# SysCV/LiDAR_snow_sim

Measured on NVIDIA H100. Metric: augmented LiDAR points/sec, higher is better.
Workload: dtype f64

## Files before the change

### lidar_snow_sim_b200/csrc/beam.cuh

```cuda
#pragma once
#include "common.cuh"

struct __align__(16) SolveItem {
    unsigned long long key;
    int hit_off;
    int L;
    float th32;
    float px, py, pz;
};

struct DevArgs {
    const ParticleRec *rec;
    const ParticleTan *tan;
    const int64_t *plane_off;
    float zbase;
    const BroadEntry *entries;
    const int32_t *bucket_start;
    int n_buckets;
    int n_planes;
    double inv_w, w;
    const float *pts;
    const float *theta;
    const int64_t *cloud_off;
    const int32_t *order;
    const double *thresh;
    const SensorConst *sensor;
    const CameraConst *camera;
    const double *R;
    const double2 *wtab;
    double half_div;
    double div_rad;
    uint32_t flags;
    float *aug;
    float *keep_d;
    float *keep_i;
    uint8_t *keep_tag;
    uint8_t *code_keep;
    uint8_t *code_all;
    int32_t *nocc;
    unsigned *hist_keep;
    unsigned *hist_all;
    const int32_t *tile_base;
    double *stats;
    int *counters;
    unsigned *att_cnt;
    unsigned long long *att_sum;
    int *status;
    SolveItem *items;
    int *chunk_tab;
    int chunks_per_class;
    int *hdr;
    int *hit_idx;
    int hit_cap;
    const unsigned long long *sched;
    int n_wtiles;
};

namespace {

constexpr int SNOW_TPB = 128;
constexpr int SNOW_WARPS = SNOW_TPB / 32;
constexpr int TILE = 1024;
constexpr int NBINS = LSS_N_CHANNELS + 1;
constexpr int LIST_HDR_BYTES = 1024;
constexpr int LIST_CLASSES = 128;
constexpr int LIST_CHUNK = 1024;
constexpr int SCHED_PLANES = 64;
constexpr int SCHED_BINS = SCHED_PLANES + 1;

__device__ __forceinline__ void raise_status(int *status, int code) { atomicMax(status, code); }

__device__ __forceinline__ int channel_bin(float ch)
{
    int c = (int)ch;
    return (ch >= 0.0f && ch < 64.0f && (float)c == ch) ? c : LSS_N_CHANNELS;
}

__device__ __forceinline__ uint8_t keep_tag_of(int bin, float label)
{
    return (uint8_t)(bin + NBINS * (label == 2.0f ? 2 : (label == 1.0f ? 1 : 0)));
}

__device__ __forceinline__ int keep_tag_label(int tag) { return tag >= 2 * NBINS ? 2 : (tag >= NBINS ? 1 : 0); }

__device__ __forceinline__ bool within(double diff, double tol)
{
    return (fabs(diff) < tol) || (fabs(diff - LSS_TWO_PI) < tol) || (fabs(diff + LSS_TWO_PI) < tol);
}

__device__ __forceinline__ double xsi64(double r)
{
    if (r <= 0.9) return 0.0;
    if (r >= 1.0) return 1.0;
    const double m = (1 - 0) / (1.0 - 0.9);
    const double b = 0 - (m * 0.9);
    return __dadd_rn(__dmul_rn(m, r), b);
}

__device__ __forceinline__ double xsi32(float r)
{
    if (r <= 0.9f) return 0.0;
    if (r >= 1.0f) return 1.0;
    const double m = (1 - 0) / (1.0 - 0.9);
    const double b = 0 - (m * 0.9);
    return (double)__fadd_rn(__fmul_rn((float)m, r), (float)b);
}


__device__ __noinline__ float azimuth32_slow(float y, float x)
{
    return (float)atan2((double)y, (double)x);
}

__device__ const double ATAN_I32[33] = {
        0.0, 0.031239833430268277, 0.06241880999595735, 0.09347678115858947,
        0.12435499454676144, 0.15499674192394097, 0.18534794999569476, 0.21535769969773805,
        0.24497866312686414, 0.2741674511196588, 0.3028848683749714, 0.3310960767041321,
        0.35877067027057225, 0.38588266939807375, 0.4124104415973873, 0.43833655985795783,
        0.4636476090008061, 0.48833395105640554, 0.5123894603107377, 0.5358112379604637,
        0.5585993153435624, 0.5807563535676704, 0.6022873461349642, 0.6231993299340659,
        0.6435011087932844, 0.6632029927060933, 0.6823165548747481, 0.7008544078844502,
        0.7188299996216245, 0.7362574289814281, 0.7531512809621944, 0.7695264804056583,
        0.7853981633974483};

__device__ __forceinline__ float azimuth32(float yf, float xf)
{
    const float axf = fabsf(xf), ayf = fabsf(yf);
    const float mxf = fmaxf(axf, ayf), mnf = fminf(axf, ayf);
    if (!(mnf > 0.0f) || !(mxf < 3.0e38f) || !(mnf > mxf * 1e-30f) || xf != xf || yf != yf) return azimuth32_slow(yf, xf);
    const int i = (int)rintf(__fdividef(mnf, mxf) * 32.0f);
    const double c = (double)i * (1.0 / 32.0), mx = (double)mxf, mn = (double)mnf;
    const double t = fma(-c, mx, mn) / fma(c, mn, mx);
    const double t2 = t * t;
    double p = fma(t2, 1.0 / 9.0, -1.0 / 7.0);
    p = fma(t2, p, 1.0 / 5.0);
// ... 17 lines not shown
```

### lidar_snow_sim_b200/csrc/snowfall.cu

```cuda
#include "beam.cuh"

namespace {

constexpr int SCHED_KEY_TPB = 128;

__global__ void __launch_bounds__(SCHED_KEY_TPB) k_sched_key(const float *__restrict__ pts, const int64_t *__restrict__ cloud_off,
                                                            const int32_t *__restrict__ order, const int32_t *__restrict__ wtile_base,
                                                            unsigned long long *ent, int *hist)
{
    const int b = blockIdx.y, t = blockIdx.x * SCHED_KEY_TPB + threadIdx.x;
    const int64_t beg = cloud_off[b];
    const int n = (int)(cloud_off[b + 1] - beg);
    if (blockIdx.x * SCHED_KEY_TPB * 32 >= n) return;
    const int w0 = 32 * t;
    const bool on = w0 < n;
    int bin = -1;
    if (on) {
        const int ch = channel_bin(pts[(beg + w0) * 5 + 4]);
        bin = ch < LSS_N_CHANNELS ? order[b * LSS_N_CHANNELS + ch] % SCHED_PLANES : SCHED_PLANES;
        ent[wtile_base[b] + t] = ((unsigned long long)bin << 48) | ((unsigned long long)b << 32) | (unsigned)w0;
    }
    const unsigned m = __match_any_sync(0xffffffffu, bin);
    if (on && (threadIdx.x & 31) == __ffs(m) - 1) atomicAdd(&hist[bin], __popc(m));
}

constexpr int HIT_POS_PER_BEAM = 6;
constexpr int SCHED_PER_THREAD = 2;
__global__ void __launch_bounds__(256) k_sched_sort(const unsigned long long *__restrict__ in, unsigned long long *out,
                                                    int *hist, int n)
{
    __shared__ int base[SCHED_BINS], cnt[SCHED_BINS], blk[SCHED_BINS];
    const int first = blockIdx.x * (256 * SCHED_PER_THREAD);
    for (int c = threadIdx.x; c < SCHED_BINS; c += 256) cnt[c] = 0;
    if (threadIdx.x < 32) {
        int run = 0;
        for (int c0 = 0; c0 < SCHED_BINS; c0 += 32) {
            const int c = c0 + (int)threadIdx.x;
            const int v = c < SCHED_BINS ? hist[c] : 0;
            int incl = v;
#pragma unroll
            for (int s = 1; s < 32; s <<= 1) {
                const int t = __shfl_up_sync(0xffffffffu, incl, s);
                if ((int)threadIdx.x >= s) incl += t;
            }
            if (c < SCHED_BINS) base[c] = run + incl - v;
            run += __shfl_sync(0xffffffffu, incl, 31);
        }
    }
    __syncthreads();
    const int lane = threadIdx.x & 31;
    int bin_of[SCHED_PER_THREAD], rank[SCHED_PER_THREAD];
    unsigned long long e[SCHED_PER_THREAD];
#pragma unroll
    for (int k = 0; k < SCHED_PER_THREAD; k++) {
        const int s = first + k * 256 + threadIdx.x;
        const bool on = s < n;
        e[k] = on ? in[s] : 0ull;
        const int bin = on ? (int)(e[k] >> 48) : -1;
        bin_of[k] = bin;
        const unsigned m = __match_any_sync(0xffffffffu, bin);
        const int leader = __ffs(m) - 1;
        int r = 0;
        if (on && lane == leader) r = atomicAdd(&cnt[bin], __popc(m));
        r = __shfl_sync(0xffffffffu, r, leader);
        rank[k] = r + __popc(m & ((1u << lane) - 1u));
    }
    __syncthreads();
    for (int c = threadIdx.x; c < SCHED_BINS; c += 256)
        blk[c] = cnt[c] ? atomicAdd(&hist[SCHED_BINS + c], cnt[c]) : 0;
    __syncthreads();
#pragma unroll
    for (int k = 0; k < SCHED_PER_THREAD; k++)
        if (bin_of[k] >= 0) out[base[bin_of[k]] + blk[bin_of[k]] + rank[k]] = e[k];
}

constexpr int KEEP_TPB = 256;
constexpr int KEEP_ROWS = TILE / KEEP_TPB;

__global__ void __launch_bounds__(KEEP_TPB) k_keep(DevArgs a)
{
    __shared__ unsigned h_keep[NBINS], h_all[NBINS];
    __shared__ int s_cnt[2];
    const int b = blockIdx.y, tile = blockIdx.x;
    const int64_t beg = a.cloud_off[b];
    const int n = (int)(a.cloud_off[b + 1] - beg);
    if (tile * TILE >= n) return;
    if (threadIdx.x < NBINS) { h_keep[threadIdx.x] = 0; h_all[threadIdx.x] = 0; }
    if (threadIdx.x < 2) s_cnt[threadIdx.x] = 0;
    const bool thr_on = a.flags & LSS_FLAG_THRESHOLD_FILTER;
    int tags[KEEP_ROWS];
    float d32s[KEEP_ROWS], out_is[KEEP_ROWS];
#pragma unroll
    for (int k = 0; k < KEEP_ROWS; k++) {
        const int i = tile * TILE + k * KEEP_TPB + threadIdx.x;
        tags[k] = 0; d32s[k] = 0.0f; out_is[k] = 0.0f;
        if (i < n) {
            tags[k] = __ldcs(a.keep_tag + beg + i);
            if (thr_on) { d32s[k] = __ldcs(a.keep_d + beg + i); out_is[k] = __ldcs(a.keep_i + beg + i); }
        }
    }
    double p0 = 0.0, p1 = 0.0, p2 = 0.0;
    if (thr_on) { p0 = a.thresh[3 * b]; p1 = a.thresh[3 * b + 1]; p2 = a.thresh[3 * b + 2]; }
    __syncthreads();
    const int lane = threadIdx.x & 31;
#pragma unroll
    for (int k = 0; k < KEEP_ROWS; k++) {
        const int i = tile * TILE + k * KEEP_TPB + threadIdx.x;
        const bool active = i < n;
        bool keep = false, att = false;
// ... 78 lines not shown
            run += __shfl_sync(0xffffffffu, incl, 31);
        }
        if (lane == 0) bin_total[c] = run;
    }
    __syncthreads();
    if (threadIdx.x == 0) {
        unsigned run = 0;
        for (int c = 0; c < NBINS; c++) { const unsigned t = bin_total[c]; bin_total[c] = run; run += t; }
        if (counts) counts[b] = (int32_t)run;
        if (stats) {
            const int n_att = counters[2 * b], n_rem = counters[2 * b + 1];
            double sum = 0.0;
            for (int c = 0; c < LSS_N_CHANNELS; c++) sum += att_term[c];
            sum -= (double)att_sum[b];
            stats[4 * b + 3] = sum;
            stats[4 * b + 0] = (double)n_att;
            stats[4 * b + 1] = (double)n_rem;
            stats[4 * b + 2] = n_att > 0 ? (double)(long long)(sum / (double)n_att) : 0.0;
        }
    }
    __syncthreads();
    const int total = n_tiles * NBINS;
    for (int k0 = threadIdx.x; k0 < total; k0 += TSCAN_ADD * blockDim.x) {
        unsigned v[TSCAN_ADD];
#pragma unroll
        for (int q = 0; q < TSCAN_ADD; q++) {
            const int k = k0 + q * blockDim.x;
            v[q] = k < total ? h[k] : 0u;
        }
#pragma unroll
        for (int q = 0; q < TSCAN_ADD; q++) {
            const int k = k0 + q * blockDim.x;
            if (k < total) h[k] = v[q] + bin_total[k % NBINS];
        }
    }
}

__global__ void __launch_bounds__(TILE) k_scatter(const float *__restrict__ aug, const uint8_t *__restrict__ code,
                                                   const unsigned *__restrict__ tile_off,
                                                   const int64_t *__restrict__ cloud_off,
                                                   const int32_t *__restrict__ tile_base,
                                                   float *__restrict__ out, const int32_t *__restrict__ nocc_in,
                                                   int32_t *__restrict__ nocc_out, int32_t *__restrict__ perm_out)
{
    __shared__ unsigned warp_cnt[TILE / 32][NBINS];
    const int b = blockIdx.y, tile = blockIdx.x;
    const int64_t beg = cloud_off[b];
    const int n = (int)(cloud_off[b + 1] - beg);
    const int i = tile * TILE + threadIdx.x;
    if (tile * TILE >= n) return;
    const int lane = threadIdx.x & 31, warp = threadIdx.x >> 5;
    for (int k = threadIdx.x; k < (TILE / 32) * NBINS; k += TILE) (&warp_cnt[0][0])[k] = 0;
    __syncthreads();
    int c = -1;
    if (i < n) {
        const int cc = code[beg + i];
        c = cc < NBINS ? cc : -1;
    }
    const unsigned m = __match_any_sync(0xffffffffu, c);
    const int rank = __popc(m & ((1u << lane) - 1u));
    if (c >= 0 && rank == 0) warp_cnt[warp][c] = __popc(m);
    __syncthreads();
    if (threadIdx.x < NBINS) {
        unsigned run = tile_off[((size_t)tile_base[b] + tile) * NBINS + threadIdx.x];
        for (int wv = 0; wv < TILE / 32; wv++) { const unsigned t = warp_cnt[wv][threadIdx.x]; warp_cnt[wv][threadIdx.x] = run; run += t; }
    }
    __syncthreads();
    if (c >= 0) {
        const int64_t dst = beg + warp_cnt[warp][c] + rank;
        const float *s = aug + (beg + i) * 5;
        float *o = out + dst * 5;
#pragma unroll
        for (int q = 0; q < 5; q++) o[q] = s[q];
        if (nocc_out) nocc_out[dst] = nocc_in[beg + i];
        if (perm_out) perm_out[dst] = i;
    }
}

struct WsLayout {
    int64_t aug, keep_d, keep_i, keep_tag, code_keep, code_all, nocc, hist_keep, hist_all, hist_rows, cloud_off, tile_base,
        order, thresh, counters, counters_bytes, list, chunks_per_class, chunk_tab, sched, sched_tiles, prepass, prepass_bytes, total;
};

WsLayout ws_layout(int64_t n_total, int n_clouds)
{
    WsLayout w;
    w.hist_rows = n_total / TILE + (int64_t)n_clouds + 1;
    w.sched_tiles = n_total / 32 + (int64_t)n_clouds + 1;
    int64_t o = 0;
    w.aug = o;        o = align_up(o + n_total * 5 * 4, 256);
    w.keep_d = o;     o = align_up(o + n_total * 4, 256);
    w.keep_i = o;     o = align_up(o + n_total * 4, 256);
    w.keep_tag = o;   o = align_up(o + n_total, 256);
    w.code_keep = o;  o = align_up(o + n_total, 256);
    w.code_all = o;   o = align_up(o + n_total, 256);
    w.nocc = o;       o = align_up(o + n_total * 4, 256);
    w.hist_keep = o;  o = align_up(o + w.hist_rows * NBINS * 4, 256);
    w.hist_all = o;   o = align_up(o + w.hist_rows * NBINS * 4, 256);
    w.cloud_off = o;  o = align_up(o + (int64_t)(n_clouds + 1) * 8, 256);
    w.tile_base = o;  o = align_up(o + (int64_t)(n_clouds + 1) * 2 * 4, 256);
    w.order = o;      o = align_up(o + (int64_t)n_clouds * LSS_N_CHANNELS * 4, 256);
    w.thresh = o;     o = align_up(o + (int64_t)n_clouds * 3 * 8, 256);
    w.counters_bytes = align_up((int64_t)n_clouds * 2 * 4, 8) + (int64_t)n_clouds * LSS_N_CHANNELS * 4 + (int64_t)n_clouds * 8;
    w.counters = o;   o = align_up(o + w.counters_bytes, 256);
    w.chunks_per_class = (n_total + LIST_CHUNK - 1) / LIST_CHUNK;
    w.list = o;       o = align_up(o + LIST_HDR_BYTES +
                                   (w.chunks_per_class + LIST_CLASSES) * LIST_CHUNK * (int64_t)sizeof(SolveItem) +
                                   (n_total * HIT_POS_PER_BEAM + 4096) * 4, 256);
    w.chunk_tab = o;  o = align_up(o + (int64_t)LIST_CLASSES * w.chunks_per_class * 4, 256);
    w.sched = o;      o = align_up(o + (int64_t)SCHED_BINS * 2 * 4 + 2 * w.sched_tiles * 8, 256);
    w.prepass_bytes = lss_prepass_ws_bytes(n_total, n_clouds);
    w.prepass = o;    o = align_up(o + w.prepass_bytes, 256);
    w.total = o;
    return w;
}

}

int64_t lss_snowfall_ws_bytes(int64_t n_total, int n_clouds)
{
    if (n_total < 0 || n_clouds < 0) return -1;
    return ws_layout(n_total, n_clouds).total;
}

int64_t lss_snowfall_ws_cloud_off(int64_t n_total, int n_clouds) { return ws_layout(n_total, n_clouds).cloud_off; }

lss_status lss_snowfall_run(lss_engine *e, const SnowfallArgs &s, cudaStream_t stream)
{
    const int B = s.n_clouds;
    BatchGeometry g, wg;
    if (lss_status rc = lss_batch_geometry(e, s.h_cloud_offsets, B, TILE, g)) return rc;
    if (lss_status rc = lss_batch_geometry(e, s.h_cloud_offsets, B, 32, wg)) return rc;
    const int64_t N = g.n, max_n = g.max_n;
    for (int k = 0; k < B * LSS_N_CHANNELS; k++)
        if (s.h_order[k] < 0 || s.h_order[k] >= s.ts->n_planes)
            return lss_fail(e, LSS_ERR_NO_TABLE, "order[] names a plane that is not in the table set");
    const WsLayout w = ws_layout(N, B);
    if (s.workspace_bytes < w.total || !s.d_workspace) return lss_fail(e, LSS_ERR_WORKSPACE, "workspace too small");
    if ((s.flags & LSS_FLAG_THRESHOLD_FILTER) && !s.h_thresh_poly && !(s.flags & LSS_FLAG_DEVICE_PREPASS))
        return lss_fail(e, LSS_ERR_INVALID_ARG, "threshold filter needs h_thresh_poly or LSS_FLAG_DEVICE_PREPASS");
    if ((s.flags & LSS_FLAG_CAMERA_FOV) && !e->has_camera)
        return lss_fail(e, LSS_ERR_NO_SENSOR, "camera calibration not set");
    const double div_rad = s.beam_divergence_deg * (LSS_PI / 180.0);
    if (!(div_rad > 0) || div_rad > s.ts->max_div_rad * (1 + 1e-12))
        return lss_fail(e, LSS_ERR_INVALID_ARG, "beam_divergence exceeds the value the table set was built for");
    const int max_tiles = (int)((max_n + TILE - 1) / TILE);
    const int n_wtiles = wg.tile_base[B];
    if ((s.d_out_perm || s.d_out_nocc) && !s.d_out_full)
        return lss_fail(e, LSS_ERR_INVALID_ARG, "d_out_perm / d_out_nocc need d_out_full");

    char *ws = (char *)s.d_workspace;
    float *d_aug = (float *)(ws + w.aug);
    uint8_t *d_code_keep = (uint8_t *)(ws + w.code_keep);
    const bool want_all = s.d_out_full != nullptr;
    uint8_t *d_code_all = want_all ? (uint8_t *)(ws + w.code_all) : nullptr;
    int32_t *d_nocc_tmp = s.d_out_nocc ? (int32_t *)(ws + w.nocc) : nullptr;
    unsigned *d_hist_keep = (unsigned *)(ws + w.hist_keep);
    unsigned *d_hist_all = want_all ? (unsigned *)(ws + w.hist_all) : nullptr;
    int64_t *d_off = (int64_t *)(ws + w.cloud_off);
    int32_t *d_tile_base = (int32_t *)(ws + w.tile_base);
    int32_t *d_order = (int32_t *)(ws + w.order);
    double *d_thresh = (double *)(ws + w.thresh);
    int *d_counters = (int *)(ws + w.counters);
    unsigned *d_att_cnt = (unsigned *)(ws + w.counters + align_up((int64_t)B * 2 * 4, 8));
    unsigned long long *d_att_sum = (unsigned long long *)((char *)d_att_cnt + (int64_t)B * LSS_N_CHANNELS * 4);

    g.tile_base.insert(g.tile_base.end(), wg.tile_base.begin(), wg.tile_base.end());
    LSS_CUDA_CHECK(e, lss_stage_geometry(e, s.h_cloud_offsets, B, g.tile_base, d_off, d_tile_base, stream));
    LSS_CUDA_CHECK(e, lss_stage_upload(e, d_order, s.h_order, sizeof(int32_t) * B * LSS_N_CHANNELS, stream));
    if (s.h_thresh_poly)
        LSS_CUDA_CHECK(e, lss_stage_upload(e, d_thresh, s.h_thresh_poly, sizeof(double) * 3 * B, stream));
    int *d_list_hdr = (int *)(ws + w.list);
    {
        ZeroRegions z;
        z.add(d_counters, w.counters_bytes);
        z.add(s.d_out_stats, sizeof(double) * 4 * B);
        if (N == 0 || B == 0) {
            z.add(s.d_out_counts, sizeof(int32_t) * B);
            LSS_CUDA_CHECK(e, lss_zero_async(e, z, stream));
            return LSS_OK;
        }
        z.add(d_list_hdr, LIST_HDR_BYTES);
        z.add(ws + w.chunk_tab, (size_t)LIST_CLASSES * w.chunks_per_class * 4);
        z.add(ws + w.sched, (size_t)SCHED_BINS * 2 * 4);
        LSS_CUDA_CHECK(e, lss_zero_async(e, z, stream));
    }

    DevArgs a;
    a.rec = s.ts->d_rec;
    a.tan = s.ts->d_tan;
    a.plane_off = s.ts->d_plane_off;
    a.zbase = s.ts->zbase;
    a.entries = s.ts->d_entries;
    a.bucket_start = s.ts->d_bucket_start;
    a.n_buckets = s.ts->n_buckets;
    a.n_planes = s.ts->n_planes;
    a.w = LSS_TWO_PI / s.ts->n_buckets;
    a.inv_w = s.ts->n_buckets / LSS_TWO_PI;
    a.pts = s.d_points;
    a.theta = s.d_theta;
    a.cloud_off = d_off;
    a.order = d_order;
    a.thresh = d_thresh;
    a.sensor = e->d_sensor;
    a.camera = e->d_camera;
    a.R = e->d_R;
    a.wtab = e->d_wtab;
    a.half_div = (s.beam_divergence_deg / 2) * (LSS_PI / 180.0);
    a.div_rad = div_rad;
    a.flags = s.flags;
    a.aug = d_aug;
    a.keep_d = (float *)(ws + w.keep_d);
    a.keep_i = (float *)(ws + w.keep_i);
    a.keep_tag = (uint8_t *)(ws + w.keep_tag);
    a.code_keep = d_code_keep;
    a.code_all = d_code_all;
    a.nocc = d_nocc_tmp;
    a.hist_keep = d_hist_keep;
    a.hist_all = d_hist_all;
    a.tile_base = d_tile_base;
    a.stats = s.d_out_stats;
    a.counters = d_counters;
    a.att_cnt = d_att_cnt;
    a.att_sum = d_att_sum;
    a.status = e->d_status;
    SolveItem *d_solve_list = (SolveItem *)(ws + w.list + LIST_HDR_BYTES);
    a.hit_idx = (int *)(d_solve_list + (w.chunks_per_class + LIST_CLASSES) * LIST_CHUNK);
    const bool device_prepass = (s.flags & LSS_FLAG_THRESHOLD_FILTER) && (s.flags & LSS_FLAG_DEVICE_PREPASS) &&
                                !s.h_thresh_poly;
    cudaEvent_t ev_join = nullptr;
    if (device_prepass) {
        cudaStream_t side = nullptr;
        cudaEvent_t ev_fork = nullptr;
        LSS_CUDA_CHECK(e, lss_side_stream(e, &side, &ev_fork, &ev_join));
        LSS_CUDA_CHECK(e, cudaEventRecord(ev_fork, stream));
        LSS_CUDA_CHECK(e, cudaStreamWaitEvent(side, ev_fork, 0));
        PrepassIO io;
        io.h_plane_in = s.h_plane_in;
        io.h_ymins_in = s.h_ymins_in;
        io.d_poly_out = d_thresh;
        lss_status ps = lss_prepass_run(e, s.d_points, d_off, nullptr, s.h_cloud_offsets, B, 0.5, s.noise_floor, 0, 0, 1,
                                io, ws + w.prepass, w.prepass_bytes, nullptr, side);
        const cudaError_t je = cudaEventRecord(ev_join, side);
        if (ps != LSS_OK || je != cudaSuccess) {
            cudaStreamWaitEvent(stream, ev_join, 0);
            return ps != LSS_OK ? ps : lss_fail(e, LSS_ERR_CUDA, "event record failed");
        }
    }
    a.hit_cap = (int)std::min<int64_t>(N * HIT_POS_PER_BEAM + 4096, 0x7fffffff);
    cudaError_t ce;
    {
        KernelTimer kt(e, LSS_K_SNOWFALL, stream);
        a.hdr = d_list_hdr;
        a.items = d_solve_list;
        a.chunk_tab = (int *)(ws + w.chunk_tab);
        a.chunks_per_class = (int)w.chunks_per_class;
        {
            int *d_sched_hist = (int *)(ws + w.sched);
            unsigned long long *d_ent = (unsigned long long *)(d_sched_hist + 2 * SCHED_BINS);
            unsigned long long *d_sched = d_ent + w.sched_tiles;
            const int max_wtiles = (int)((max_n + 31) / 32);
            ce = lss_launch(e, k_sched_key, dim3((unsigned)((max_wtiles + SCHED_KEY_TPB - 1) / SCHED_KEY_TPB), (unsigned)B),
                            SCHED_KEY_TPB, 0, stream, s.d_points, d_off, d_order, d_tile_base + B + 1, d_ent, d_sched_hist);
            if (ce == cudaSuccess)
                ce = lss_launch(e, k_sched_sort, (unsigned)((n_wtiles + 256 * SCHED_PER_THREAD - 1) / (256 * SCHED_PER_THREAD)),
                                256, 0, stream, d_ent, d_sched, d_sched_hist, n_wtiles);
            a.sched = d_sched;
            a.n_wtiles = n_wtiles;
        }
        if (ce == cudaSuccess) {
            KernelTimer ks(e, LSS_K_SCAN, stream);
            ce = lss_launch_scan(e, a, stream);
        }
        if (ce == cudaSuccess) {
            KernelTimer ks(e, LSS_K_SOLVE, stream);
            ce = lss_launch_solve(e, a, d_list_hdr + 1, stream);
        }
    }
    if (ev_join) LSS_CUDA_CHECK(e, cudaStreamWaitEvent(stream, ev_join, 0));
    LSS_CUDA_CHECK(e, ce);
    {
        KernelTimer kt(e, LSS_K_FINALIZE, stream);
        LSS_CUDA_CHECK(e, lss_launch(e, k_keep, dim3(max_tiles, B), KEEP_TPB, 0, stream, a));
    }
    {
        KernelTimer kt(e, LSS_K_SORT, stream);
        LSS_CUDA_CHECK(e, lss_launch(e, k_tile_scan, B, 1024, 0, stream, d_hist_keep, d_tile_base, s.d_out_counts,
                                     s.d_out_stats, d_counters, d_att_cnt, d_att_sum, e->d_sensor));
    }
    {
        KernelTimer kt(e, LSS_K_COMPACT, stream);
        LSS_CUDA_CHECK(e, lss_launch(e, k_scatter, dim3(max_tiles, B), TILE, 0, stream, d_aug, d_code_keep, d_hist_keep, d_off,
                                     d_tile_base, s.d_out_points, nullptr, nullptr, nullptr));
    }
    if (want_all) {
        KernelTimer kt(e, LSS_K_COMPACT, stream);
        LSS_CUDA_CHECK(e, lss_launch(e, k_tile_scan, B, 1024, 0, stream, d_hist_all, d_tile_base, nullptr, nullptr, nullptr,
                                     nullptr, nullptr, nullptr));
        LSS_CUDA_CHECK(e, lss_launch(e, k_scatter, dim3(max_tiles, B), TILE, 0, stream, d_aug, d_code_all, d_hist_all, d_off,
                                     d_tile_base, s.d_out_full, d_nocc_tmp, s.d_out_nocc, s.d_out_perm));
    }
    return LSS_OK;
}
```

### lidar_snow_sim_b200/csrc/solve.cu

```cuda
#include "beam.cuh"

namespace {

constexpr int SOLVE_TPB = 128;
constexpr int SOLVE_WARPS = SOLVE_TPB / 32;
#ifndef LSS_SOLVE_CTAS
#define LSS_SOLVE_CTAS 5
#endif
#ifndef LSS_SOLVE_ARENA
#define LSS_SOLVE_ARENA 160
#endif
constexpr int SOLVE_CTAS_PER_SM = LSS_SOLVE_CTAS;
constexpr int ARENA = LSS_SOLVE_ARENA;
constexpr int SOLVE_LCAP = 128;
static_assert(SOLVE_LCAP + 1 <= ARENA, "a beam with SOLVE_LCAP occluders must fit a round of the arena on its own");
constexpr unsigned FULL = 0xffffffffu;

struct Beam {
    double d, right, left;
    bool straddle;
};

__device__ __forceinline__ void beam_limits(float th32, double half_div, Beam &bm)
{
    const double thd = (double)th32;
    double right = thd - half_div, left = thd + half_div;
    if (right < 0) right += LSS_TWO_PI;
    if (left < 0) left += LSS_TWO_PI;
    if (right > LSS_TWO_PI) right -= LSS_TWO_PI;
    if (left > LSS_TWO_PI) left -= LSS_TWO_PI;
    bm.right = right; bm.left = left; bm.straddle = right > left;
}

__device__ __forceinline__ bool exact_hit(const ParticleRec *rp, const Beam &bm, double &rho, bool &right_hit, bool &left_hit)
{
    rho = rp->rho;
    if (!(rho < bm.d)) return false;
    const double phi = rp->phi, alpha = rp->alpha;
    bool inside = (bm.right <= phi) && (phi <= bm.left);
    if (bm.straddle) inside = inside || ((bm.right - LSS_TWO_PI <= phi) && (phi <= bm.left)) ||
                              ((bm.right <= phi) && (phi <= bm.left + LSS_TWO_PI));
    right_hit = within(bm.right - phi, alpha);
    left_hit = within(bm.left - phi, alpha);
    return inside || right_hit || left_hit;
}

struct Bucket {
    int e0, e1;
    float th_rel;
    long long pbase;
};

__device__ __forceinline__ Bucket beam_bucket(const DevArgs &a, int plane, float th32)
{
    const double thd = (double)th32;
    const double thm = thd >= LSS_TWO_PI ? thd - LSS_TWO_PI : thd;
    int bk = (int)(thm * a.inv_w);
    bk = bk < 0 ? 0 : (bk >= a.n_buckets ? a.n_buckets - 1 : bk);
    const int32_t *bs = a.bucket_start + (int64_t)plane * (a.n_buckets + 1) + bk;
    Bucket k;
    k.e0 = bs[0];
    k.e1 = bs[1];
    k.th_rel = (float)(thm - (bk + 0.5) * a.w);
    k.pbase = a.plane_off[plane];
    return k;
}

template <class F>
__device__ __forceinline__ int for_each_hit(const DevArgs &a, const Bucket &k, const Beam &bm, float d32, F &&f)
{
    int n = 0;
#pragma unroll 1
    for (int e = k.e0; e < k.e1; e++) {
        const EntryView en = lss_decode(__ldg(&a.entries[e]), a.zbase);
        if (!(en.x < d32)) break;
        if (!(fabsf(en.y - k.th_rel) <= en.z)) continue;
        const long long pi = k.pbase + en.idx;
        double rho;
        bool rh, lh;
        if (exact_hit(a.rec + pi, bm, rho, rh, lh)) { f((int)pi, rho, rh, lh); n++; }
    }
    return n;
}

constexpr int SURV_CAP = 20;

__device__ __forceinline__ double shfl_f64(double v, int src)
{
    const long long b = __double_as_longlong(v);
    const int lo = __shfl_sync(FULL, (int)(unsigned)b, src), hi = __shfl_sync(FULL, (int)(b >> 32), src);
    return __longlong_as_double(((long long)hi << 32) | (unsigned)lo);
}

#ifndef LSS_SCAN_CTAS
#define LSS_SCAN_CTAS 10
#endif
__global__ void __launch_bounds__(SNOW_TPB, LSS_SCAN_CTAS) k_scan(DevArgs a)
{
    __shared__ float s_rows[SNOW_WARPS][32 * 5];
    __shared__ int s_idx[SNOW_WARPS][32][SURV_CAP];
    __shared__ unsigned s_hit[SNOW_WARPS][32];
    const int lane = threadIdx.x & 31, wid = threadIdx.x >> 5;
    const int st = blockIdx.x * SNOW_WARPS + wid;
    if (st >= a.n_wtiles) return;
    const unsigned long long se = a.sched[st];
    const int b = (int)((se >> 32) & 0xffffu), w0 = (int)(unsigned)se;
    const int64_t beg = a.cloud_off[b];
    const int n = (int)(a.cloud_off[b + 1] - beg);
    const int i = w0 + lane;
    const bool active = i < n;
    const int nf_w = min(32, n - w0) * 5;
    float px = 0, py = 0, pz = 0, pint = 0, pch = 0;
    {
        const float *src = a.pts + (beg + w0) * 5;
#pragma unroll
        for (int q = 0; q < 5; q++) {
            const int f = q * 32 + lane;
            if (f < nf_w) s_rows[wid][f] = __ldcs(src + f);
        }
        __syncwarp();
        if (active) {
            const float *row = &s_rows[wid][5 * lane];
            px = row[0]; py = row[1]; pz = row[2]; pint = row[3]; pch = row[4];
        }
    }
    const float d32 = __fsqrt_rn(__fadd_rn(__fadd_rn(__fmul_rn(px, px), __fmul_rn(py, py)), __fmul_rn(pz, pz)));
    const int ch = channel_bin(pch);
    float out_l = pch;
    int ns = 0;
    Bucket bkt;
    bkt.e0 = bkt.e1 = 0; bkt.th_rel = 0.0f; bkt.pbase = 0;
    bool slow = false;
    float th32 = 0.0f;
    Beam bm;
    bm.d = (double)d32; bm.right = bm.left = 0.0; bm.straddle = false;
    if (active && ch < LSS_N_CHANNELS) {
        out_l = 0.0f;
        th32 = a.theta ? a.theta[beg + i] : azimuth32(py, px);
        if (th32 < 0.0f) th32 = __fadd_rn(th32, 6.2831855f);
        beam_limits(th32, a.half_div, bm);
        const int plane = a.order[b * LSS_N_CHANNELS + ch];
        if (plane >= 0 && plane < a.n_planes && th32 == th32) {
            bkt = beam_bucket(a, plane, th32);
            const int e1 = bkt.e1;
            int *pos = s_idx[wid][lane];
            bool stop = false;
#pragma unroll 1
            for (int e = bkt.e0; e < e1 && !stop; e += 4) {
                BroadEntry raw[4];
#pragma unroll
                for (int q = 0; q < 4; q++) raw[q] = __ldg(&a.entries[min(e + q, e1 - 1)]);
#pragma unroll
                for (int q = 0; q < 4; q++) {
                    if (stop || e + q >= e1) continue;
                    const EntryView en = lss_decode(raw[q], a.zbase);
                    if (!(en.x < d32)) { stop = true; continue; }
                    if (!(fabsf(en.y - bkt.th_rel) <= en.z)) continue;
                    if (ns < SURV_CAP) pos[ns] = en.idx;
                    else slow = true;
                    ns++;
                }
            }
        }
    }
    s_hit[wid][lane] = 0u;
    const int mine = slow ? 0 : ns;
    int incl = mine;
#pragma unroll
    for (int sft = 1; sft < 32; sft <<= 1) {
        const int t = __shfl_up_sync(FULL, incl, sft);
        if (lane >= sft) incl += t;
    }
    const int off = incl - mine;
    const int total = __shfl_sync(FULL, incl, 31);
    __syncwarp();
#pragma unroll 1
    for (int s0 = 0; s0 < total; s0 += 32) {
        const int s = s0 + lane;
        int j = 0;
#pragma unroll
        for (int step = 16; step; step >>= 1) {
            const int c = j + step;
            const int oc = __shfl_sync(FULL, off, c & 31);
            if (c < 32 && oc <= s) j = c;
        }
        const int r = s - __shfl_sync(FULL, off, j);
        const long long pbj = __shfl_sync(FULL, bkt.pbase, j);
        Beam bj;
        bj.d = shfl_f64(bm.d, j);
        bj.right = shfl_f64(bm.right, j);
        bj.left = shfl_f64(bm.left, j);
        bj.straddle = bj.right > bj.left;
        if (s < total) {
            double rho;
            bool rh, lh;
            if (exact_hit(a.rec + pbj + s_idx[wid][j][r], bj, rho, rh, lh)) atomicOr(&s_hit[wid][j], 1u << r);
        }
    }
    __syncwarp();
    unsigned hits = s_hit[wid][lane];
    int L = __popc(hits);
    if (slow) L = for_each_hit(a, bkt, bm, d32, [](int, double, bool, bool) {});
    {
        const bool push = L > 0;
        const unsigned pm = __ballot_sync(FULL, push);
        int lincl = push ? L : 0;
#pragma unroll
        for (int sft = 1; sft < 32; sft <<= 1) {
            const int t = __shfl_up_sync(FULL, lincl, sft);
            if (lane >= sft) lincl += t;
        }
        const int ltotal = __shfl_sync(FULL, lincl, 31);
        if (pm) {
            int hbase = 0;
            const int leader = __ffs(pm) - 1;
            if (lane == leader) hbase = atomicAdd(a.hdr + 2, ltotal);
            hbase = __shfl_sync(FULL, hbase, leader);
            if (push) {
                const int cls = LIST_CLASSES - 1 - min(LIST_CLASSES - 1, 2 * min(L, 63) + (d32 > 40.0f ? 1 : 0));
                const unsigned cm = __match_any_sync(pm, cls);
                const int cl = __ffs(cm) - 1;
                int j = 0;
                if (lane == cl) j = atomicAdd(a.hdr + LIST_CLASSES + cls, __popc(cm));
                j = __shfl_sync(cm, j, cl) + __popc(cm & ((1u << lane) - 1u));
                int *ct = a.chunk_tab + (int64_t)cls * a.chunks_per_class + j / LIST_CHUNK;
                if (j % LIST_CHUNK == 0) atomicExch(ct, atomicAdd(a.hdr, 1) + 1);
                __syncwarp(pm);
                int chunk;
                while ((chunk = *(volatile int *)ct) == 0) {}
                const int hoff = hbase + lincl - L;
                const bool fits = hoff + L <= a.hit_cap;
                {
                    SolveItem it;
                    it.key = ((unsigned long long)ch << 56) | ((unsigned long long)cls << 48) |
                             ((unsigned long long)b << 32) | (unsigned)i;
                    it.hit_off = fits ? hoff : -1;
                    it.L = L;
                    it.th32 = th32;
                    it.px = px;
                    it.py = py;
                    it.pz = pz;
                    a.items[(int64_t)(chunk - 1) * LIST_CHUNK + j % LIST_CHUNK] = it;
                }
                if (fits) {
                    int *hp = a.hit_idx + hoff;
                    if (!slow) {
                        const int *pos = s_idx[wid][lane];
#pragma unroll 1
                        for (int k = 0; hits; hits &= hits - 1) hp[k++] = (int)bkt.pbase + pos[__ffs(hits) - 1];
                    } else {
                        for_each_hit(a, bkt, bm, d32, [&](int pi, double, bool, bool) { *hp++ = pi; });
                    }
                }
            }
        }
    }
    __syncwarp();
    if (active) {
        float *row = &s_rows[wid][5 * lane];
        const float out_i = rintf(pint);
        row[3] = out_i;
        row[4] = out_l;
        if (a.nocc) a.nocc[beg + i] = 0;
        a.keep_d[beg + i] = d32;
        a.keep_i[beg + i] = out_i;
        a.keep_tag[beg + i] = (uint8_t)ch;
    }
    __syncwarp();
    {
        float *dst = a.aug + (beg + w0) * 5;
#pragma unroll
        for (int q = 0; q < 5; q++) {
            const int f = q * 32 + lane;
            if (f < nf_w) dst[f] = s_rows[wid][f];
        }
    }
}

__device__ __forceinline__ unsigned long long pack_win(int ks, int ke, int k0)
{
    return (unsigned long long)(unsigned)ks | ((unsigned long long)(unsigned)ke << 11) | ((unsigned long long)(unsigned)k0 << 22);
}

__device__ __forceinline__ void pulse_phase(double r, double &sb, double &cb)
{
    const double ctau = 299792458.0 * 1e-8, inv_ctau = 1.0 / (299792458.0 * 1e-8);
    const double bh = r * inv_ctau;
    const double bl = fma(-bh, ctau, r) * inv_ctau;
    double s, c;
    sincospi(bh, &s, &c);
    const double corr = LSS_PI * bl;
    sb = fma(corr, c, s);
    cb = fma(-corr, s, c);
}

__device__ __forceinline__ void cp_async4(void *dst, const void *src)
{
    asm volatile("cp.async.ca.shared.global [%0], [%1], 4;\n" ::"r"((unsigned)__cvta_generic_to_shared(dst)), "l"(src) : "memory");
}
__device__ __forceinline__ void cp_async8(void *dst, const void *src)
{
    asm volatile("cp.async.ca.shared.global [%0], [%1], 8;\n" ::"r"((unsigned)__cvta_generic_to_shared(dst)), "l"(src) : "memory");
}
__device__ __forceinline__ void cp_async_wait_all() { asm volatile("cp.async.wait_all;\n" ::: "memory"); }

#ifdef LSS_SOLVE_PHASE_CLOCKS
enum { PH_FETCH, PH_FILL, PH_CLAIM, PH_PULSES, PH_SWEEP, PH_EVAL, PH_STORE, PH_N };
static_assert(PH_N + 2 + LIST_CLASSES == LSS_DEBUG_SOLVE_PHASE_WORDS, "layout of lss_debug_solve_phases");
__device__ unsigned long long g_solve_phase[LSS_DEBUG_SOLVE_PHASE_WORDS];
#define PHASE_INIT()                                                                                                  \
    __shared__ unsigned long long s_ph[SOLVE_WARPS][PH_N + 1];                                                        \
    if (lane <= PH_N) s_ph[wid][lane] = 0ull;                                                                         \
    unsigned ph_t = (unsigned)clock64();                         \
    unsigned ph_split = 0u
#define PHASE(k)                                                                                                      \
    do {                                                                                                              \
        const unsigned ph_n = (unsigned)clock64();                                                                    \
        if (lane == 0) s_ph[wid][k] += ph_n - ph_t;                                                                   \
        ph_t = ph_n;                                                                                                  \
    } while (0)
#define PHASE_MARK() (ph_split = (unsigned)clock64() - ph_t)
#define PHASE_SPLIT(k0, k1)                                                                                           \
    do {                                                                                                              \
        const unsigned ph_n = (unsigned)clock64();                                                                    \
        const unsigned sp = __reduce_max_sync(FULL, ph_split);                                                        \
        if (lane == 0) { s_ph[wid][k0] += sp; s_ph[wid][k1] += ph_n - ph_t - sp; }                                   \
        ph_t = ph_n;                                                                                                  \
        ph_split = 0u;                                                                                                \
    } while (0)
#define PHASE_TILE(cls, active)                                                                                       \
    do {                                                                                                              \
        const unsigned nb = __popc(__ballot_sync(FULL, active));                                                      \
        if (lane == 0) { s_ph[wid][PH_N]++; atomicAdd(&g_solve_phase[PH_N + 2 + (cls)], (unsigned long long)nb); }    \
    } while (0)
#define PHASE_FLUSH()                                                                                                 \
    do {                                                                                                              \
        if (lane <= PH_N) atomicAdd(&g_solve_phase[lane], s_ph[wid][lane]);                                           \
        if (lane == 0) atomicAdd(&g_solve_phase[PH_N + 1], 1ull);                                                     \
    } while (0)
#else
#define PHASE_INIT()
#define PHASE(k)
#define PHASE_MARK()
#define PHASE_SPLIT(k0, k1)
#define PHASE_TILE(cls, active)
#define PHASE_FLUSH()
#endif

__global__ void __launch_bounds__(SOLVE_TPB, SOLVE_CTAS_PER_SM) k_solve(DevArgs a, int *tile_cursor)
{
    __shared__ double s_arena[SOLVE_WARPS][4][ARENA];
    __shared__ unsigned long long s_piece[SOLVE_WARPS][2 * ARENA];
    __shared__ int s_piece_k[SOLVE_WARPS][2 * ARENA];
    const int lane = threadIdx.x & 31, wid = threadIdx.x >> 5;
    unsigned long long *PD = s_piece[wid];
    int *PK = s_piece_k[wid];
    double *A0 = s_arena[wid][0], *A1 = s_arena[wid][1], *A2 = s_arena[wid][2], *A3 = s_arena[wid][3];
    unsigned long long *W = reinterpret_cast<unsigned long long *>(A2);

    __shared__ int s_tile0[LIST_CLASSES + 1];
    __shared__ int s_cnt[LIST_CLASSES];
    if (wid == 0) {
        int run = 0;
        for (int c0 = 0; c0 < LIST_CLASSES; c0 += 32) {
            const int n = a.hdr[LIST_CLASSES + c0 + lane];
            s_cnt[c0 + lane] = n;
            const int v = (n + 31) >> 5;
            int incl = v;
#pragma unroll
            for (int sft = 1; sft < 32; sft <<= 1) {
                const int t = __shfl_up_sync(FULL, incl, sft);
                if (lane >= sft) incl += t;
            }
            s_tile0[c0 + lane] = run + incl - v;
            run += __shfl_sync(FULL, incl, 31);
        }
        if (lane == 0) s_tile0[LIST_CLASSES] = run;
    }
    __syncthreads();
    const int n_tiles = s_tile0[LIST_CLASSES];
    const double ctau = 299792458.0 * 1e-8;
    const double inv_step = (double)(LSS_M_EXT - 1) / (120 + ctau);
// ... 13 lines not shown
        SolveItem e;
        e.key = 0ull; e.hit_off = 0; e.L = 0; e.th32 = 0.0f; e.px = 0.0f; e.py = 0.0f; e.pz = 0.0f;
        return e;
    };
    int tile = 0;
    if (lane == 0) tile = atomicAdd(tile_cursor, 1);
    tile = __shfl_sync(FULL, tile, 0);
    SolveItem it = empty_item();
    {
        int c, j;
        if (beam_of(tile, c, j)) it = item_of(chunk_of(c, j), j);
    }

    while (tile < n_tiles) {
        int cls, jn;
        const bool active = beam_of(tile, cls, jn);
        int nxt = 0;
        if (lane == 0) nxt = atomicAdd(tile_cursor, 1);
        int nchunk = 0;
        bool fetched = false;
        SolveItem nx = empty_item();
        const auto next_chunk = [&] {
            nxt = __shfl_sync(FULL, nxt, 0);
            if (beam_of(nxt, cls, jn)) nchunk = chunk_of(cls, jn);
        };
        const auto next_item = [&] {
            if (nchunk > 0) nx = item_of(nchunk, jn);
            fetched = true;
        };
        const int b = (int)((it.key >> 32) & 0xffffu);
        const int i = (int)(it.key & 0xffffffffu);
        const int ch = (int)(it.key >> 56);
        const int64_t beg = a.cloud_off[b];
        const float px = it.px, py = it.py, pz = it.pz;
        const float d32 = __fsqrt_rn(__fadd_rn(__fadd_rn(__fmul_rn(px, px), __fmul_rn(py, py)), __fmul_rn(pz, pz)));

        float out_x = px, out_y = py, out_z = pz, out_i = 0.0f, out_l = 0.0f;
        long long att_new_i = -1;
        int n_claim = 0;

        const int L = active ? it.L : 0;
        Beam bm;
        bm.d = (double)d32;
        beam_limits(it.th32, a.half_div, bm);

        if (L > SOLVE_LCAP) raise_status(a.status, LSS_ERR_OCCLUDER_OVERFLOW);
        const int need = (L > 0 && L <= SOLVE_LCAP) ? L + 1 : 0;
        PHASE_TILE(cls, active);
        PHASE(PH_FETCH);

        unsigned remaining = __ballot_sync(FULL, need > 0);
        while (remaining) {
            const bool rem = (remaining >> lane) & 1u;
            const int mine = rem ? need : 0;
            int incl = mine;
#pragma unroll
            for (int s = 1; s < 32; s <<= 1) {
                const int t = __shfl_up_sync(FULL, incl, s);
                if (lane >= s) incl += t;
            }
            const bool in_round = rem && incl <= ARENA;
            remaining &= ~__ballot_sync(FULL, in_round);
            const int off = incl - mine;
            const int total = (int)__reduce_max_sync(FULL, in_round ? (unsigned)incl : 0u);
            int n_pulses = 0;
            double amax = 0.0;
            double best = 0.0;
            int kbest = 0;

#pragma unroll 1
            for (int s0 = 0; s0 < total; s0 += 32) {
                const int s = s0 + lane;
                int j = 0;
#pragma unroll
                for (int step = 16; step; step >>= 1) {
                    const int c = j + step;
                    const int oc = __shfl_sync(FULL, off, c & 31);
                    if (c < 32 && oc <= s) j = c;
                }
                const int r = s - __shfl_sync(FULL, off, j);
                const int Lj = __shfl_sync(FULL, L, j);
                const int hoj = __shfl_sync(FULL, it.hit_off, j);
                const int inr = __shfl_sync(FULL, (int)in_round, j);
                if (s < total) {
                    PK[ARENA + s] = j;
                    if (inr && r < Lj && hoj >= 0) cp_async4(&PK[s], &a.hit_idx[hoj + r]);
                    else PK[s] = -1;
                }
            }
            cp_async_wait_all();
            __syncwarp();
#pragma unroll 1
            for (int s = lane; s < total; s += 32) {
                const int pi = PK[s];
                if (pi >= 0) {
                    cp_async8(&A0[s], &a.rec[pi].phi);
                    cp_async8(&A1[s], &a.rec[pi].rho);
                    cp_async8(&A2[s], &a.rec[pi].alpha);
                    cp_async8(&A3[s], &a.tan[pi].t_right);
                    cp_async8(&PD[s], &a.tan[pi].t_left);
                }
            }
            cp_async_wait_all();
            __syncwarp();
#pragma unroll 1
            for (int s0 = 0; s0 < total; s0 += 32) {
                const int s = s0 + lane;
                const int j = s < total ? PK[ARENA + s] : 0;
                Beam bj;
                bj.d = shfl_f64(bm.d, j);
                bj.right = shfl_f64(bm.right, j);
                bj.left = shfl_f64(bm.left, j);
                bj.straddle = bj.right > bj.left;
                if (s < total && PK[s] >= 0) {
                    ParticleRec rc;
                    rc.phi = A0[s]; rc.rho = A1[s]; rc.alpha = A2[s];
                    double rho;
                    bool rh, lh;
                    exact_hit(&rc, bj, rho, rh, lh);
                    A0[s] = rh ? bj.right : A3[s];
                    A1[s] = lh ? bj.left : __longlong_as_double((long long)PD[s]);
                    A2[s] = rho;
                }
            }
            if (in_round && it.hit_off < 0) {
                const Bucket bkt = beam_bucket(a, a.order[b * LSS_N_CHANNELS + ch], it.th32);
                int s = off;
                for_each_hit(a, bkt, bm, d32, [&](int pi, double rho, bool rh, bool lh) {
                    A0[s] = rh ? bm.right : a.tan[pi].t_right;
                    A1[s] = lh ? bm.left : a.tan[pi].t_left;
                    A2[s] = rho;
                    s++;
                });
            }
            __syncwarp();
            if (!fetched) next_chunk();
            PHASE(PH_FILL);

            if (in_round) {
#pragma unroll 1
                for (int p = 1; p < L; p++) {
                    const double rho = A2[off + p];
                    if (!(A2[off + p - 1] > rho)) continue;
                    const double a1 = A0[off + p], a2 = A1[off + p];
                    int q = p - 1;
#pragma unroll 1
                    while (q >= 0 && A2[off + q] > rho) { A0[off + q + 1] = A0[off + q]; A1[off + q + 1] = A1[off + q]; A2[off + q + 1] = A2[off + q]; q--; }
                    A0[off + q + 1] = a1; A1[off + q + 1] = a2; A2[off + q + 1] = rho;
                }

                double rb = bm.right;
                if (bm.straddle) rb = bm.right - LSS_TWO_PI;
                int nu = 0, P = 0;
                double ep_min = fmin(rb, bm.left), ep_max = fmax(rb, bm.left), claimed_total = 0.0;
#pragma unroll 1
                for (int j = 0; j < L; j++) {
                    double lo = A0[off + j];
                    const double hi = A1[off + j], rho = A2[off + j];
                    if (bm.straddle && lo > hi) lo -= LSS_TWO_PI;
                    ep_min = fmin(ep_min, fmin(lo, hi));
                    ep_max = fmax(ep_max, fmax(lo, hi));
                    if (!(lo < hi)) continue;
                    bool contained = false;
                    double cov = 0.0, nlo = lo, nhi = hi;
                    int w = 0;
#pragma unroll 1
                    for (int u = 0; u < nu; u++) {
                        const double ul = A0[off + u], uh = A1[off + u];
                        if ((ul <= lo) && (hi <= uh)) { contained = true; break; }
                        if (ul <= hi && uh >= lo) {
                            const double ov = fmin(hi, uh) - fmax(lo, ul);
                            if (ov > 0.0) cov += ov;
                            nlo = fmin(nlo, ul);
                            nhi = fmax(nhi, uh);
                        } else {
                            A0[off + w] = ul; A1[off + w] = uh; w++;
                        }
                    }
                    if (contained) continue;
                    const double claimed = (hi - lo) - cov;
                    claimed_total += claimed;
                    A0[off + w] = nlo; A1[off + w] = nhi;
                    nu = w + 1;
                    double ratio = claimed / a.div_rad;
                    ratio = ratio < 0 ? 0 : (ratio > 1 ? 1 : ratio);
                    A2[off + P] = rho;
                    A3[off + P] = ratio;
                    P++;
                }
                n_claim = P;
                double ratio_hard = ((ep_max - ep_min) - claimed_total) / a.div_rad;
                ratio_hard = ratio_hard < 0 ? 0 : (ratio_hard > 1 ? 1 : ratio_hard);
                PHASE_MARK();

                if (P > 0) {
                    const double beta_0 = 1 * 1e-06 / LSS_PI;
                    const double i_orig = 0.9 * a.sensor->max_intensity[ch];
                    const double A = (i_orig / beta_0) * beta_0;
                    bool bad = false;
#pragma unroll 1
                    for (int j = 0; j < P; j++) {
                        const double r = A2[off + j], ratio = A3[off + j];
                        const int ks = (int)ceil(r * 10);
                        const int ke = (int)(floor((r + ctau) * 10) + 1);
                        bad |= (ke > LSS_M_EXT) || (ks < 0);
                        double sb, cb;
                        pulse_phase(r, sb, cb);
// ... 242 lines not shown
```

Baseline: 4.542 billion.

## Store precomputed hit angles and rho in scan instead of particle indices

The scan kernel now writes per-hit results (clipped right/left angles and rho) into three SoA double arrays, using a warp-level allocation reserved before the candidate loop. The solve kernel then loads these directly instead of fetching indices, gathering particle records and re-running the exact hit test. This removes a dependent gather stage and duplicate hit evaluation in solve. In exchange scan does more global writes (24 bytes per hit instead of 4), the workspace grows, and every candidate's tan record is read in scan whether or not it hits. Hit slots per beam drop from 6 to 3.

```diff
diff --git a/lidar_snow_sim_b200/csrc/beam.cuh b/lidar_snow_sim_b200/csrc/beam.cuh
--- a/lidar_snow_sim_b200/csrc/beam.cuh
+++ b/lidar_snow_sim_b200/csrc/beam.cuh
@@ -50,7 +50,9 @@
     int *chunk_tab;
     int chunks_per_class;
     int *hdr;
-    int *hit_idx;
+    double *hit_a1;
+    double *hit_a2;
+    double *hit_rho;
     int hit_cap;
     const unsigned long long *sched;
     int n_wtiles;
diff --git a/lidar_snow_sim_b200/csrc/snowfall.cu b/lidar_snow_sim_b200/csrc/snowfall.cu
--- a/lidar_snow_sim_b200/csrc/snowfall.cu
+++ b/lidar_snow_sim_b200/csrc/snowfall.cu
@@ -24,7 +24,7 @@
     if (on && (threadIdx.x & 31) == __ffs(m) - 1) atomicAdd(&hist[bin], __popc(m));
 }
 
-constexpr int HIT_POS_PER_BEAM = 6;
+constexpr int HIT_SLOTS_PER_BEAM = 3;
 constexpr int SCHED_PER_THREAD = 2;
 __global__ void __launch_bounds__(256) k_sched_sort(const unsigned long long *__restrict__ in, unsigned long long *out,
                                                     int *hist, int n)
@@ -269,6 +269,8 @@
         order, thresh, counters, counters_bytes, list, chunks_per_class, chunk_tab, sched, sched_tiles, prepass, prepass_bytes, total;
 };
 
+int64_t hit_cap(int64_t n_total) { return std::min<int64_t>(n_total * HIT_SLOTS_PER_BEAM + 4096, 0x7fffffff); }
+
 WsLayout ws_layout(int64_t n_total, int n_clouds)
 {
     WsLayout w;
@@ -293,7 +295,7 @@
     w.chunks_per_class = (n_total + LIST_CHUNK - 1) / LIST_CHUNK;
     w.list = o;       o = align_up(o + LIST_HDR_BYTES +
                                    (w.chunks_per_class + LIST_CLASSES) * LIST_CHUNK * (int64_t)sizeof(SolveItem) +
-                                   (n_total * HIT_POS_PER_BEAM + 4096) * 4, 256);
+                                   hit_cap(n_total) * 3 * 8, 256);
     w.chunk_tab = o;  o = align_up(o + (int64_t)LIST_CLASSES * w.chunks_per_class * 4, 256);
     w.sched = o;      o = align_up(o + (int64_t)SCHED_BINS * 2 * 4 + 2 * w.sched_tiles * 8, 256);
     w.prepass_bytes = lss_prepass_ws_bytes(n_total, n_clouds);
@@ -412,7 +414,10 @@
     a.att_sum = d_att_sum;
     a.status = e->d_status;
     SolveItem *d_solve_list = (SolveItem *)(ws + w.list + LIST_HDR_BYTES);
-    a.hit_idx = (int *)(d_solve_list + (w.chunks_per_class + LIST_CLASSES) * LIST_CHUNK);
+    a.hit_cap = (int)hit_cap(N);
+    a.hit_a1 = (double *)(d_solve_list + (w.chunks_per_class + LIST_CLASSES) * LIST_CHUNK);
+    a.hit_a2 = a.hit_a1 + a.hit_cap;
+    a.hit_rho = a.hit_a2 + a.hit_cap;
     const bool device_prepass = (s.flags & LSS_FLAG_THRESHOLD_FILTER) && (s.flags & LSS_FLAG_DEVICE_PREPASS) &&
                                 !s.h_thresh_poly;
     cudaEvent_t ev_join = nullptr;
@@ -434,7 +439,6 @@
             return ps != LSS_OK ? ps : lss_fail(e, LSS_ERR_CUDA, "event record failed");
         }
     }
-    a.hit_cap = (int)std::min<int64_t>(N * HIT_POS_PER_BEAM + 4096, 0x7fffffff);
     cudaError_t ce;
     {
         KernelTimer kt(e, LSS_K_SNOWFALL, stream);
diff --git a/lidar_snow_sim_b200/csrc/solve.cu b/lidar_snow_sim_b200/csrc/solve.cu
--- a/lidar_snow_sim_b200/csrc/solve.cu
+++ b/lidar_snow_sim_b200/csrc/solve.cu
@@ -35,14 +35,13 @@
 __device__ __forceinline__ bool exact_hit(const ParticleRec *rp, const Beam &bm, double &rho, bool &right_hit, bool &left_hit)
 {
     rho = rp->rho;
-    if (!(rho < bm.d)) return false;
     const double phi = rp->phi, alpha = rp->alpha;
-    bool inside = (bm.right <= phi) && (phi <= bm.left);
-    if (bm.straddle) inside = inside || ((bm.right - LSS_TWO_PI <= phi) && (phi <= bm.left)) ||
-                              ((bm.right <= phi) && (phi <= bm.left + LSS_TWO_PI));
+    bool inside = (bm.right <= phi) & (phi <= bm.left);
+    if (bm.straddle) inside = inside | ((bm.right - LSS_TWO_PI <= phi) & (phi <= bm.left)) |
+                              ((bm.right <= phi) & (phi <= bm.left + LSS_TWO_PI));
     right_hit = within(bm.right - phi, alpha);
     left_hit = within(bm.left - phi, alpha);
-    return inside || right_hit || left_hit;
+    return (rho < bm.d) & (inside | right_hit | left_hit);
 }
 
 struct Bucket {
@@ -84,13 +83,6 @@
 }
 
 constexpr int SURV_CAP = 20;
-
-__device__ __forceinline__ double shfl_f64(double v, int src)
-{
-    const long long b = __double_as_longlong(v);
-    const int lo = __shfl_sync(FULL, (int)(unsigned)b, src), hi = __shfl_sync(FULL, (int)(b >> 32), src);
-    return __longlong_as_double(((long long)hi << 32) | (unsigned)lo);
-}
 
 #ifndef LSS_SCAN_CTAS
 #define LSS_SCAN_CTAS 10
@@ -110,7 +102,7 @@
     const int i = w0 + lane;
     const bool active = i < n;
     const int nf_w = min(32, n - w0) * 5;
-    float px = 0, py = 0, pz = 0, pint = 0, pch = 0;
+    float px = 0, py = 0, pz = 0, pch = 0;
     {
         const float *src = a.pts + (beg + w0) * 5;
 #pragma unroll
@@ -121,7 +113,7 @@
         __syncwarp();
         if (active) {
             const float *row = &s_rows[wid][5 * lane];
-            px = row[0]; py = row[1]; pz = row[2]; pint = row[3]; pch = row[4];
+            px = row[0]; py = row[1]; pz = row[2]; pch = row[4];
         }
     }
     const float d32 = __fsqrt_rn(__fadd_rn(__fadd_rn(__fmul_rn(px, px), __fmul_rn(py, py)), __fmul_rn(pz, pz)));
@@ -132,13 +124,10 @@
     bkt.e0 = bkt.e1 = 0; bkt.th_rel = 0.0f; bkt.pbase = 0;
     bool slow = false;
     float th32 = 0.0f;
-    Beam bm;
-    bm.d = (double)d32; bm.right = bm.left = 0.0; bm.straddle = false;
     if (active && ch < LSS_N_CHANNELS) {
         out_l = 0.0f;
         th32 = a.theta ? a.theta[beg + i] : azimuth32(py, px);
         if (th32 < 0.0f) th32 = __fadd_rn(th32, 6.2831855f);
-        beam_limits(th32, a.half_div, bm);
         const int plane = a.order[b * LSS_N_CHANNELS + ch];
         if (plane >= 0 && plane < a.n_planes && th32 == th32) {
             bkt = beam_bucket(a, plane, th32);
@@ -173,6 +162,8 @@
     }
     const int off = incl - mine;
     const int total = __shfl_sync(FULL, incl, 31);
+    int hbase = 0;
+    if (lane == 0 && total > 0) hbase = atomicAdd(a.hdr + 2, total);
     __syncwarp();
 #pragma unroll 1
     for (int s0 = 0; s0 < total; s0 += 32) {
@@ -184,81 +175,84 @@
             const int oc = __shfl_sync(FULL, off, c & 31);
             if (c < 32 && oc <= s) j = c;
         }
-        const int r = s - __shfl_sync(FULL, off, j);
+        const int off_j = __shfl_sync(FULL, off, j);
+        const int r = s - off_j;
         const long long pbj = __shfl_sync(FULL, bkt.pbase, j);
         Beam bj;
-        bj.d = shfl_f64(bm.d, j);
-        bj.right = shfl_f64(bm.right, j);
-        bj.left = shfl_f64(bm.left, j);
-        bj.straddle = bj.right > bj.left;
+        bj.d = (double)__shfl_sync(FULL, d32, j);
+        beam_limits(__shfl_sync(FULL, th32, j), a.half_div, bj);
+        bool hit = false;
+        double rho = 0.0, a1 = 0.0, a2 = 0.0;
         if (s < total) {
-            double rho;
+            const long long pi = pbj + s_idx[wid][j][r];
+            const ParticleTan tn = a.tan[pi];
             bool rh, lh;
-            if (exact_hit(a.rec + pbj + s_idx[wid][j][r], bj, rho, rh, lh)) atomicOr(&s_hit[wid][j], 1u << r);
+            hit = exact_hit(a.rec + pi, bj, rho, rh, lh);
+            a1 = rh ? bj.right : tn.t_right;
+            a2 = lh ? bj.left : tn.t_left;
+            if (hit) atomicOr(&s_hit[wid][j], 1u << r);
+        }
+        const int region = __shfl_sync(FULL, hbase, 0) + off_j;
+        const bool stored = region + (__shfl_sync(FULL, incl, j) - off_j) <= a.hit_cap;
+        __syncwarp();
+        if (hit && stored) {
+            const int k = region + __popc(s_hit[wid][j] & ((1u << r) - 1u));
+            a.hit_a1[k] = a1;
+            a.hit_a2[k] = a2;
+            a.hit_rho[k] = rho;
         }
     }
     __syncwarp();
-    unsigned hits = s_hit[wid][lane];
-    int L = __popc(hits);
+    hbase = __shfl_sync(FULL, hbase, 0);
+    int L = __popc(s_hit[wid][lane]);
+    Beam bm;
+    bm.d = (double)d32;
+    beam_limits(th32, a.half_div, bm);
     if (slow) L = for_each_hit(a, bkt, bm, d32, [](int, double, bool, bool) {});
     {
         const bool push = L > 0;
         const unsigned pm = __ballot_sync(FULL, push);
-        int lincl = push ? L : 0;
-#pragma unroll
-        for (int sft = 1; sft < 32; sft <<= 1) {
-            const int t = __shfl_up_sync(FULL, lincl, sft);
-            if (lane >= sft) lincl += t;
-        }
-        const int ltotal = __shfl_sync(FULL, lincl, 31);
-        if (pm) {
-            int hbase = 0;
-            const int leader = __ffs(pm) - 1;
-            if (lane == leader) hbase = atomicAdd(a.hdr + 2, ltotal);
-            hbase = __shfl_sync(FULL, hbase, leader);
-            if (push) {
-                const int cls = LIST_CLASSES - 1 - min(LIST_CLASSES - 1, 2 * min(L, 63) + (d32 > 40.0f ? 1 : 0));
-                const unsigned cm = __match_any_sync(pm, cls);
-                const int cl = __ffs(cm) - 1;
-                int j = 0;
-                if (lane == cl) j = atomicAdd(a.hdr + LIST_CLASSES + cls, __popc(cm));
-                j = __shfl_sync(cm, j, cl) + __popc(cm & ((1u << lane) - 1u));
-                int *ct = a.chunk_tab + (int64_t)cls * a.chunks_per_class + j / LIST_CHUNK;
-                if (j % LIST_CHUNK == 0) atomicExch(ct, atomicAdd(a.hdr, 1) + 1);
-                __syncwarp(pm);
-                int chunk;
-                while ((chunk = *(volatile int *)ct) == 0) {}
-                const int hoff = hbase + lincl - L;
-                const bool fits = hoff + L <= a.hit_cap;
-                {
-                    SolveItem it;
-                    it.key = ((unsigned long long)ch << 56) | ((unsigned long long)cls << 48) |
-                             ((unsigned long long)b << 32) | (unsigned)i;
-                    it.hit_off = fits ? hoff : -1;
-                    it.L = L;
-                    it.th32 = th32;
-                    it.px = px;
-                    it.py = py;
-                    it.pz = pz;
-                    a.items[(int64_t)(chunk - 1) * LIST_CHUNK + j % LIST_CHUNK] = it;
-                }
-                if (fits) {
-                    int *hp = a.hit_idx + hoff;
-                    if (!slow) {
-                        const int *pos = s_idx[wid][lane];
-#pragma unroll 1
-                        for (int k = 0; hits; hits &= hits - 1) hp[k++] = (int)bkt.pbase + pos[__ffs(hits) - 1];
-                    } else {
-                        for_each_hit(a, bkt, bm, d32, [&](int pi, double, bool, bool) { *hp++ = pi; });
-                    }
-                }
+        if (push) {
+            const int cls = LIST_CLASSES - 1 - min(LIST_CLASSES - 1, 2 * min(L, 63) + (d32 > 40.0f ? 1 : 0));
+            const unsigned cm = __match_any_sync(pm, cls);
+            const int cl = __ffs(cm) - 1;
+            int j = 0;
+            if (lane == cl) j = atomicAdd(a.hdr + LIST_CLASSES + cls, __popc(cm));
+            j = __shfl_sync(cm, j, cl) + __popc(cm & ((1u << lane) - 1u));
+            int *ct = a.chunk_tab + (int64_t)cls * a.chunks_per_class + j / LIST_CHUNK;
+            if (j % LIST_CHUNK == 0) atomicExch(ct, atomicAdd(a.hdr, 1) + 1);
+            __syncwarp(pm);
+            int chunk;
+            while ((chunk = *(volatile int *)ct) == 0) {}
+            const int hoff = slow ? atomicAdd(a.hdr + 2, L) : hbase + off;
+            const bool fits = hoff + (slow ? L : mine) <= a.hit_cap;
+            {
+                SolveItem it;
+                it.key = ((unsigned long long)ch << 56) | ((unsigned long long)cls << 48) |
+                         ((unsigned long long)b << 32) | (unsigned)i;
+                it.hit_off = fits ? hoff : -1;
+                it.L = L;
+                it.th32 = th32;
+                it.px = s_rows[wid][5 * lane];
+                it.py = s_rows[wid][5 * lane + 1];
+                it.pz = s_rows[wid][5 * lane + 2];
+                a.items[(int64_t)(chunk - 1) * LIST_CHUNK + j % LIST_CHUNK] = it;
+            }
+            if (fits && slow) {
+                int k = hoff;
+                for_each_hit(a, bkt, bm, d32, [&](int pi, double rho, bool rh, bool lh) {
+                    a.hit_a1[k] = rh ? bm.right : a.tan[pi].t_right;
+                    a.hit_a2[k] = lh ? bm.left : a.tan[pi].t_left;
+                    a.hit_rho[k] = rho;
+                    k++;
+                });
             }
         }
     }
     __syncwarp();
     if (active) {
         float *row = &s_rows[wid][5 * lane];
-        const float out_i = rintf(pint);
+        const float out_i = rintf(row[3]);
         row[3] = out_i;
         row[4] = out_l;
         if (a.nocc) a.nocc[beg + i] = 0;
@@ -294,10 +288,6 @@
     cb = fma(-corr, s, c);
 }
 
-__device__ __forceinline__ void cp_async4(void *dst, const void *src)
-{
-    asm volatile("cp.async.ca.shared.global [%0], [%1], 4;\n" ::"r"((unsigned)__cvta_generic_to_shared(dst)), "l"(src) : "memory");
-}
 __device__ __forceinline__ void cp_async8(void *dst, const void *src)
 {
     asm volatile("cp.async.ca.shared.global [%0], [%1], 8;\n" ::"r"((unsigned)__cvta_generic_to_shared(dst)), "l"(src) : "memory");
@@ -477,47 +467,14 @@
                 const int Lj = __shfl_sync(FULL, L, j);
                 const int hoj = __shfl_sync(FULL, it.hit_off, j);
                 const int inr = __shfl_sync(FULL, (int)in_round, j);
-                if (s < total) {
-                    PK[ARENA + s] = j;
-                    if (inr && r < Lj && hoj >= 0) cp_async4(&PK[s], &a.hit_idx[hoj + r]);
-                    else PK[s] = -1;
+                if (s < total && inr && r < Lj && hoj >= 0) {
+                    cp_async8(&A0[s], &a.hit_a1[hoj + r]);
+                    cp_async8(&A1[s], &a.hit_a2[hoj + r]);
+                    cp_async8(&A2[s], &a.hit_rho[hoj + r]);
                 }
             }
             cp_async_wait_all();
             __syncwarp();
-#pragma unroll 1
-            for (int s = lane; s < total; s += 32) {
-                const int pi = PK[s];
-                if (pi >= 0) {
-                    cp_async8(&A0[s], &a.rec[pi].phi);
-                    cp_async8(&A1[s], &a.rec[pi].rho);
-                    cp_async8(&A2[s], &a.rec[pi].alpha);
-                    cp_async8(&A3[s], &a.tan[pi].t_right);
-                    cp_async8(&PD[s], &a.tan[pi].t_left);
-                }
-            }
-            cp_async_wait_all();
-            __syncwarp();
-#pragma unroll 1
-            for (int s0 = 0; s0 < total; s0 += 32) {
-                const int s = s0 + lane;
-                const int j = s < total ? PK[ARENA + s] : 0;
-                Beam bj;
-                bj.d = shfl_f64(bm.d, j);
-                bj.right = shfl_f64(bm.right, j);
-                bj.left = shfl_f64(bm.left, j);
-                bj.straddle = bj.right > bj.left;
-                if (s < total && PK[s] >= 0) {
-                    ParticleRec rc;
-                    rc.phi = A0[s]; rc.rho = A1[s]; rc.alpha = A2[s];
-                    double rho;
-                    bool rh, lh;
-                    exact_hit(&rc, bj, rho, rh, lh);
-                    A0[s] = rh ? bj.right : A3[s];
-                    A1[s] = lh ? bj.left : __longlong_as_double((long long)PD[s]);
-                    A2[s] = rho;
-                }
-            }
             if (in_round && it.hit_off < 0) {
                 const Bucket bkt = beam_bucket(a, a.order[b * LSS_N_CHANNELS + ch], it.th32);
                 int s = off;
```

Result: faster. 4.761 billion, median of 6 (+4.8%).
